# NVlabs/latentfusion

Hardware: AMD Instinct MI355X
Metric: pose-optim iters/sec (reconstruct+render+backward), 16 views, 128^3 voxels (higher is better)
Workload: dtype f32

## Files before the change

### latentfusion_amd/csrc/conv.hip

```cpp
#include "lf_common.h"

namespace {

constexpr int TX = 16;

template <int DIMS> struct TileGeom;
template <> struct TileGeom<3> { static constexpr int TY = 4, TZ = 4, HY = 6, HZ = 6, TAPS = 27; };
template <> struct TileGeom<2> { static constexpr int TY = 16, TZ = 1, HY = 18, HZ = 1, TAPS = 9; };

template <int NT, int NR, bool WHOLE = false>
__device__ __forceinline__ void epilogue_store(f32x4 (&acc)[NT][NR], const long (&rowoff)[NR], const long (&rowidx)[NR],
                                               const float* __restrict__ bias, float* __restrict__ y,
                                               float* __restrict__ norm_out, int Cout, int co_base,
                                               int ysc, long yss, bool vec_out,
                                               float he, unsigned flags, float slope, float eps,
                                               const float* __restrict__ prev_y = nullptr,
                                               const float* __restrict__ prev_norm = nullptr, unsigned prev_flags = 0,
                                               float* __restrict__ amax_out = nullptr) {
  float lane_amax = 0.f;
  const int lane = threadIdx.x & 63;
  const int cq = lane >> 4;
  float bv[NT][4];
#pragma unroll
  for (int t = 0; t < NT; ++t)
// ... 310 lines not shown
#pragma unroll
  for (int j = 0; j < 4; ++j) {
    const int r = wave * 4 + j;
    const int gy = y0 + ((DIMS == 3) ? (r & 3) : r);
    const int gz = (DIMS == 3) ? z0 + (r >> 2) : 0;
    const int gx = x0 + li;
    rowidx[j] = (gx < W && gy < H && gz < D) ? ((((long)n * D + gz) * H + gy) * W + gx) : -1;
    rowoff[j] = rowidx[j] < 0 ? -1 : rowidx[j] * Cout;
  }
  epilogue_store<1, 4>(acc, rowoff, rowidx, bias, y, norm_out, Cout, 0, 1 << 30, 0, (Cout & 3) == 0,
                       he, flags, slope, eps, prev_y, prev_norm, prev_flags);
}

namespace p3 {
constexpr int TZ = 4, TY = 8, HZ = 6, HY = 10, HX = TX + 2;
constexpr int HALO = HZ * HY * HX;
constexpr int NTHREADS = 512;
constexpr int NSLOT = (HALO * 4 + 63) / 64;
constexpr int NIT = (NSLOT + 7) / 8;
constexpr int BUF_FLOATS = NSLOT * 256;
}

__global__ void __launch_bounds__(512, 2) conv3d_c16_persistent_kernel(
    const float* __restrict__ x, const float* __restrict__ wpack, const float* __restrict__ bias,
    float* __restrict__ y, float* __restrict__ norm_out,
    int N, int D, int H, int W, int tiles_x, int tiles_y, int tiles_z, int ntiles,
    float he, unsigned flags, float slope, float eps,
    const float* __restrict__ prev_y, const float* __restrict__ prev_norm, unsigned prev_flags) {
  __shared__ __attribute__((aligned(16))) float lds[2 * p3::BUF_FLOATS];

  const int tid = threadIdx.x, lane = tid & 63;
  const int wave = __builtin_amdgcn_readfirstlane(tid >> 6);
  const int li = lane & 15, cq = lane >> 4;

  const int per = (ntiles + gridDim.x - 1) / gridDim.x;
  const int t_begin = blockIdx.x * per;
  const int t_end = min(t_begin + per, ntiles);
  if (t_begin >= t_end) return;

  const long nvox = (long)D * H * W;
  const unsigned sample_bytes = (unsigned)(nvox * 64);

  int rel[p3::NIT];
  int lxyz[p3::NIT];
#pragma unroll
  for (int it = 0; it < p3::NIT; ++it) {
    const int e = (wave + 8 * it) * 64 + lane;
    int v = e >> 2;
    const int q = e & 3;
    const int lx = v % p3::HX; v /= p3::HX;
    const int ly = v % p3::HY;
    const int lz = v / p3::HY;
    const bool inside = e < p3::HALO * 4;
    rel[it] = ((lz * H + ly) * W + lx) * 64 + q * 16;
    lxyz[it] = inside ? (lx | (ly << 8) | (lz << 16)) : 0x7f7f7f;
  }

  f32x4 wreg[27];
  {
    const float* wl = wpack + li * 16 + cq * 4;
#pragma unroll
    for (int tap = 0; tap < 27; ++tap) wreg[tap] = *(const f32x4*)(wl + tap * 256);
  }
  f32x4 bv4 = (f32x4){0.f, 0.f, 0.f, 0.f};
  if (bias != nullptr) bv4 = *(const f32x4*)(bias + cq * 4);

  int rowoffs[4];
#pragma unroll
  for (int j = 0; j < 4; ++j) {
    const int r = wave * 4 + j;
    rowoffs[j] = (((r >> 3) * p3::HY + (r & 7)) * p3::HX + li) * 16 + cq * 4;
  }

  auto issue_dma = [&](int t, int buf) {
    int tt = t;
    const int bx = tt % tiles_x; tt /= tiles_x;
    const int by = tt % tiles_y; tt /= tiles_y;
    const int bz = tt % tiles_z; tt /= tiles_z;
    const int n = tt;
    const int ox = bx * TX - 1, oy = by * p3::TY - 1, oz = bz * p3::TZ - 1;
    const int tile_off = ((oz * H + oy) * W + ox) * 64;
    __amdgpu_buffer_rsrc_t rs = __builtin_amdgcn_make_buffer_rsrc((void*)(x + (long)n * nvox * 16), 0,
                                                                  sample_bytes, 0x00020000);
#pragma unroll
    for (int it = 0; it < p3::NIT; ++it) {
      const int s = wave + 8 * it;
      if (s < p3::NSLOT) {
        const int gx = ox + (lxyz[it] & 0xff), gy = oy + ((lxyz[it] >> 8) & 0xff), gz = oz + (lxyz[it] >> 16);
        const bool ok = (unsigned)gx < (unsigned)W && (unsigned)gy < (unsigned)H && (unsigned)gz < (unsigned)D;
        const int voff = ok ? (rel[it] + tile_off) : 0x7fffffff;
        __builtin_amdgcn_raw_ptr_buffer_load_lds(
            rs, (__attribute__((address_space(3))) void*)(lds + buf * p3::BUF_FLOATS + s * 256), 16, voff, 0, 0, 0);
      }
    }
  };

  issue_dma(t_begin, 0);
  asm volatile("s_waitcnt vmcnt(0)" ::: "memory");
  __syncthreads();

  f32x4 acc[4];

  f32x4 pyv[4];
  float pnv[4];
  auto prefetch_prev = [&](int t) {
    if (prev_y == nullptr) return;
    int tt = t;
    const int bx = tt % tiles_x; tt /= tiles_x;
    const int by = tt % tiles_y; tt /= tiles_y;
    const int bz = tt % tiles_z; tt /= tiles_z;
    const float* pybase = prev_y + (long)tt * nvox * 16;
    const float* pnbase = prev_norm ? prev_norm + (long)tt * nvox : nullptr;
    const int gx = bx * TX + li;
#pragma unroll
    for (int j = 0; j < 4; ++j) {
      const int r = wave * 4 + j;
      const int gz = bz * p3::TZ + (r >> 3), gy = by * p3::TY + (r & 7);
      const bool ok = gx < W && gy < H && gz < D;
      const int vox = ok ? (gz * H + gy) * W + gx : 0;
      pyv[j] = ok ? *(const f32x4*)(pybase + vox * 16 + cq * 4) : (f32x4){0.f, 0.f, 0.f, 0.f};
      pnv[j] = (ok && pnbase) ? pnbase[vox] : 1.f;
    }
  };

  auto compute = [&](int buf) {
    const float* base = lds + buf * p3::BUF_FLOATS;
#pragma unroll
    for (int j = 0; j < 4; ++j) acc[j] = (f32x4){0.f, 0.f, 0.f, 0.f};
    f32x4 bcur[4], bnext[4];
#pragma unroll
    for (int j = 0; j < 4; ++j) bcur[j] = *(const f32x4*)(base + rowoffs[j]);
#pragma unroll
    for (int tap = 0; tap < 27; ++tap) {
      if (tap + 1 < 27) {
        const int t1 = tap + 1;
        const int kx = t1 % 3, ky = (t1 / 3) % 3, kz = t1 / 9;
        const int toff = ((kz * p3::HY + ky) * p3::HX + kx) * 16;
#pragma unroll
        for (int j = 0; j < 4; ++j) bnext[j] = *(const f32x4*)(base + rowoffs[j] + toff);
      }
#pragma unroll
      for (int s4 = 0; s4 < 4; ++s4)
#pragma unroll
        for (int j = 0; j < 4; ++j)
          acc[j] = __builtin_amdgcn_mfma_f32_16x16x4f32(wreg[tap][s4], bcur[j][s4], acc[j], 0, 0, 0);
#pragma unroll
      for (int j = 0; j < 4; ++j) bcur[j] = bnext[j];
    }
  };

  auto epilogue = [&](int t) {
    int tt = t;
    const int bx = tt % tiles_x; tt /= tiles_x;
    const int by = tt % tiles_y; tt /= tiles_y;
    const int bz = tt % tiles_z; tt /= tiles_z;
    const int n = tt;
    float* ybase = y + (long)n * nvox * 16;
    float* nbase = norm_out ? norm_out + (long)n * nvox : nullptr;
    const int gx = bx * TX + li;
#pragma unroll
    for (int j = 0; j < 4; ++j) {
      const int r = wave * 4 + j;
      const int gz = bz * p3::TZ + (r >> 3), gy = by * p3::TY + (r & 7);
      if (prev_y != nullptr) {
        const bool ok = gx < W && gy < H && gz < D;
        const int vox = ok ? (gz * H + gy) * W + gx : 0;
        const f32x4 yp = pyv[j];
        f32x4 g = acc[j] * he;
        if (prev_flags & LF_EPI_PIXELNORM) {
          float dot = g[0] * yp[0] + g[1] * yp[1] + g[2] * yp[2] + g[3] * yp[3];
          dot += __shfl_xor(dot, 16, 64);
          dot += __shfl_xor(dot, 32, 64);
          dot *= (1.f / 16.f);
          const float rinv = 1.0f / pnv[j];
#pragma unroll
          for (int e = 0; e < 4; ++e) g[e] = (g[e] - yp[e] * dot) * rinv;
        }
        if (prev_flags & LF_EPI_LRELU) {
#pragma unroll
          for (int e = 0; e < 4; ++e) g[e] = yp[e] > 0.f ? g[e] : g[e] * slope;
        }
        if (ok) *(f32x4*)(ybase + vox * 16 + cq * 4) = g;
        continue;
      }
      f32x4 v;
      float ss = 0.f;
#pragma unroll
      for (int e = 0; e < 4; ++e) {
        float u = acc[j][e] * he + bv4[e];
        if (flags & LF_EPI_LRELU) u = fmaxf(u, u * slope);
        v[e] = u;
        ss += u * u;
      }
      float r_ = 1.f;
      if (flags & LF_EPI_PIXELNORM) {
        ss += __shfl_xor(ss, 16, 64);
        ss += __shfl_xor(ss, 32, 64);
        r_ = sqrtf(ss / 16.f + eps);
        const float rinv = 1.0f / r_;
        v[0] *= rinv; v[1] *= rinv; v[2] *= rinv; v[3] *= rinv;
      }
      if (gx < W && gy < H && gz < D) {
        const int vox = (gz * H + gy) * W + gx;
        *(f32x4*)(ybase + vox * 16 + cq * 4) = v;
        if ((flags & LF_EPI_PIXELNORM) && nbase != nullptr && cq == 0) nbase[vox] = r_;
      }
    }
  };

  int cur = 0;
  if (wave < 4) {
    for (int t = t_begin; t < t_end; ++t) {
      if (t + 1 < t_end) issue_dma(t + 1, cur ^ 1);
      prefetch_prev(t);
      compute(cur);
      epilogue(t);
      asm volatile("s_waitcnt vmcnt(0)" ::: "memory");
      __syncthreads();
      cur ^= 1;
    }
  } else {
    for (int t = t_begin; t < t_end; ++t) {
      if (t + 1 < t_end) issue_dma(t + 1, cur ^ 1);
      if (t > t_begin) epilogue(t - 1);
      prefetch_prev(t);
      compute(cur);
      asm volatile("s_waitcnt vmcnt(0)" ::: "memory");
      __syncthreads();
      cur ^= 1;
    }
    epilogue(t_end - 1);
  }
}

template <int NT>
__global__ void __launch_bounds__(256) conv1x1_kernel(
    const float* __restrict__ x, const float* __restrict__ wpack, const float* __restrict__ bias,
    float* __restrict__ y, float* __restrict__ norm_out,
    int P, int Cin, int ksl, long x_batch_stride, long x_slice_stride, int Cout, int Kp,
    long y_batch_stride, int y_row_stride, int y_slice_channels, long y_slice_stride,
    float he, unsigned flags, float slope, float eps,
    const float* __restrict__ prev_y, const float* __restrict__ prev_norm, unsigned prev_flags,
    float* __restrict__ amax_out, const float* __restrict__ xscale) {
  const int tid = threadIdx.x, lane = tid & 63, wave = tid >> 6;
  const int li = lane & 15, cq = lane >> 4;
  const int n = blockIdx.z;
  const int co_base = blockIdx.y * NT * 16;
  const long p = (long)blockIdx.x * 64 + wave * 16 + li;
  const bool live = p < P;
  const bool vec_in = ((Cin & 3) == 0);
  const float* xrow = x + (long)n * x_batch_stride + (live ? p : 0) * Cin;
  const float* wrow = wpack + (long)(co_base + li) * Kp + cq * 4;

  f32x4 acc[NT][1];
#pragma unroll
  for (int t = 0; t < NT; ++t) acc[t][0] = (f32x4){0.f, 0.f, 0.f, 0.f};

  const int K = ksl * Cin;
  const int nchunks = Kp >> 4;
  auto load_b = [&](int kc) -> f32x4 {
    const int k0 = kc * 16 + cq * 4;
    f32x4 bfrag = (f32x4){0.f, 0.f, 0.f, 0.f};
    if (live && k0 < K) {
      const int s = k0 / Cin, c0 = k0 - s * Cin;
      const float* src = xrow + (long)s * x_slice_stride + c0;
      if (vec_in) {
        bfrag = *(const f32x4*)src;
        if (xscale != nullptr) bfrag = bfrag * xscale[((long)n * ksl + s) * P + p];
      } else {
#pragma unroll
        for (int e = 0; e < 4; ++e)
          if (k0 + e < K) bfrag[e] = src[e];
      }
    }
    return bfrag;
  };
  auto mac = [&](int kc, const f32x4& bfrag) {
#pragma unroll
    for (int t = 0; t < NT; ++t) {
      const f32x4 afrag = *(const f32x4*)(wrow + (long)t * 16 * Kp + kc * 16);
#pragma unroll
      for (int st = 0; st < 4; ++st)
        acc[t][0] = __builtin_amdgcn_mfma_f32_16x16x4f32(afrag[st], bfrag[st], acc[t][0], 0, 0, 0);
    }
  };
  int kc = 0;
  if (NT == 1) {
    for (; kc + 4 <= nchunks; kc += 4) {
      f32x4 b4[4];
#pragma unroll
      for (int u = 0; u < 4; ++u) b4[u] = load_b(kc + u);
#pragma unroll
      for (int u = 0; u < 4; ++u) mac(kc + u, b4[u]);
    }
  }
  for (; kc < nchunks; ++kc) mac(kc, load_b(kc));
  long rowidx[1] = {live ? ((long)n * P + p) : -1};
  long rowoff[1] = {live ? ((long)n * y_batch_stride + p * y_row_stride) : -1};
  const bool vec_out = ((y_row_stride | y_slice_channels) & 3) == 0 && ((y_batch_stride | y_slice_stride) & 3) == 0;
  epilogue_store<NT, 1>(acc, rowoff, rowidx, bias, y, norm_out, Cout, co_base, y_slice_channels, y_slice_stride,
                        vec_out, he, flags, slope, eps, prev_y, prev_norm, prev_flags, amax_out);
}

}

extern "C" int lf_conv3x3_cout_padded(int Cout) {
  lf_clear_error();
  const int c16 = (Cout + 15) & ~15;
  if (c16 <= 16) return 16;
  if (c16 <= 32) return 32;
  return (c16 + 63) & ~63;
}

extern "C" int lf_conv1x1_cout_padded(int Cout) {
  lf_clear_error();
  const int c16 = (Cout + 15) & ~15;
  if (c16 <= 16) return 16;
  if (c16 <= 32) return 32;
  if (c16 <= 64) return 64;
  return (c16 + 127) & ~127;
}

static int conv3x3_launch(const float* x, const float* wpack, const float* bias, float* y, float* norm_out,
                          int dims, int N, int D, int H, int W, int Cin, int Cout,
                          float he, unsigned flags, float slope, float eps, void* stream,
                          const float* prev_y, const float* prev_norm, unsigned prev_flags) {
  if (N <= 0 || D <= 0 || H <= 0 || W <= 0 || Cin <= 0 || Cout <= 0) return LF_EINVAL;
  if (prev_y != nullptr) {
    if (flags != 0 || bias != nullptr || (Cout != 16 && Cout != 32 && Cout != 64) || !lf_aligned16(prev_y)) return LF_EINVAL;
    if ((prev_flags & LF_EPI_PIXELNORM) && prev_norm == nullptr) return LF_EINVAL;
  }
  if (dims != 2 && dims != 3) return LF_EINVAL;
  if (dims == 2 && D != 1) return LF_EINVAL;
  if ((flags & LF_EPI_PIXELNORM) && Cout > 64) return LF_EINVAL;
  if (!lf_aligned16(x) || !lf_aligned16(y) || !lf_aligned16(wpack)) return LF_EALIGN;
  const int CinP = (Cin + 15) & ~15, CoutP = lf_conv3x3_cout_padded(Cout);
  const int ntiles = CoutP / 16;
  const int NT = ntiles >= 4 ? 4 : ntiles;
  const int groups = ntiles / NT;
  const int TY = dims == 3 ? 4 : 16, TZ = dims == 3 ? 4 : 1;
  const int tiles_x = (W + TX - 1) / TX, tiles_y = (H + TY - 1) / TY, tiles_z = (D + TZ - 1) / TZ;
  const long nblk = (long)tiles_x * tiles_y * tiles_z * N;
  if (nblk > 0x7fffffffL) return LF_EINVAL;
  dim3 grid((unsigned)nblk, groups), block(256);
  hipStream_t s = (hipStream_t)stream;
  if (Cin == 16 && Cout == 16 && dims == 3 && (long)D * H * W >= 4096 && (long)D * H * W * 64 < 0x7fffffffL &&
      slope > 0.f && slope < 1.f && (bias == nullptr || lf_aligned16(bias))) {
    const int ptx = (W + TX - 1) / TX, pty = (H + p3::TY - 1) / p3::TY, ptz = (D + p3::TZ - 1) / p3::TZ;
    const long pt = (long)ptx * pty * ptz * N;
    if (pt <= 0x7fffffffL) {
      const int cus = lf_cu_count();
      const unsigned pgrid = (unsigned)(pt < cus ? pt : cus);
      hipLaunchKernelGGL(conv3d_c16_persistent_kernel, dim3(pgrid), dim3(p3::NTHREADS), 0, s, x, wpack, bias, y, norm_out,
                         N, D, H, W, ptx, pty, ptz, (int)pt, he, flags, slope, eps, prev_y, prev_norm, prev_flags);
      return lf_launch_status();
    }
  }
  if (CinP == 16 && CoutP == 16) {
    if (dims == 3)
      hipLaunchKernelGGL((conv3x3_c16_kernel<3>), grid, block, 0, s, x, wpack, bias, y, norm_out, N, D, H, W, Cin, Cout,
                         tiles_x, tiles_y, tiles_z, he, flags, slope, eps, prev_y, prev_norm, prev_flags);
    else
      hipLaunchKernelGGL((conv3x3_c16_kernel<2>), grid, block, 0, s, x, wpack, bias, y, norm_out, N, D, H, W, Cin, Cout,
                         tiles_x, tiles_y, tiles_z, he, flags, slope, eps, prev_y, prev_norm, prev_flags);
    return lf_launch_status();
  }
#define LAUNCH(DM, T) hipLaunchKernelGGL((conv3x3_kernel<DM, T>), grid, block, 0, s, x, wpack, bias, y, norm_out, \
                                         N, D, H, W, Cin, Cout, CinP, CoutP, tiles_x, tiles_y, tiles_z, he, flags, slope, eps, \
                                         prev_y, prev_norm, prev_flags)
  if (dims == 3) { if (NT == 4) LAUNCH(3, 4); else if (NT == 2) LAUNCH(3, 2); else LAUNCH(3, 1); }
  else           { if (NT == 4) LAUNCH(2, 4); else if (NT == 2) LAUNCH(2, 2); else LAUNCH(2, 1); }
#undef LAUNCH
  return lf_launch_status();
}

extern "C" int lf_conv3x3_fwd(const float* x, const float* wpack, const float* bias, float* y, float* norm_out,
                              int dims, int N, int D, int H, int W, int Cin, int Cout,
                              float he, unsigned flags, float slope, float eps, void* stream) {
  lf_clear_error();
  return conv3x3_launch(x, wpack, bias, y, norm_out, dims, N, D, H, W, Cin, Cout, he, flags, slope, eps, stream,
                        nullptr, nullptr, 0);
}

extern "C" int lf_conv3x3_bwd_data(const float* gy, const float* wpack_t, float* gx, int dims, int N, int D, int H, int W,
                                   int Cin, int Cout, float he, const float* prev_y, const float* prev_norm,
                                   unsigned prev_flags, float slope, void* stream) {
  lf_clear_error();
  return conv3x3_launch(gy, wpack_t, nullptr, gx, nullptr, dims, N, D, H, W, Cin, Cout, he, 0, slope, 0.f, stream,
                        prev_y, prev_norm, prev_flags);
}

static int conv1x1_launch(const float* x, const float* wpack, const float* bias, float* y, float* norm_out,
                          int N, int P, int Cin, int ksl, long x_batch_stride, long x_slice_stride,
                          int Cout, long y_batch_stride, int y_row_stride, int y_slice_channels,
                          long y_slice_stride,
                          float he, unsigned flags, float slope, float eps, void* stream,
                          const float* prev_y, const float* prev_norm, unsigned prev_flags, float* amax_out = nullptr,
                          const float* xscale = nullptr) {
  if (N <= 0 || P <= 0 || Cin <= 0 || ksl <= 0 || Cout <= 0 || y_slice_channels <= 0) return LF_EINVAL;
  if (xscale != nullptr && (Cin & 3)) return LF_EALIGN;
  if (prev_y != nullptr) {
    if (flags != 0 || bias != nullptr || y_slice_channels != 16 || y_row_stride != 16 || (Cout & 15) ||
        !lf_aligned16(prev_y) || ((y_batch_stride | y_slice_stride) & 15))
      return LF_EINVAL;
    if ((prev_flags & LF_EPI_PIXELNORM) && prev_norm == nullptr) return LF_EINVAL;
    if ((prev_flags & LF_EPI_DOT) && (prev_flags != LF_EPI_DOT || prev_norm == nullptr)) return LF_EINVAL;
  }
  if (y_row_stride < (y_slice_channels < Cout ? y_slice_channels : Cout)) return LF_EINVAL;
  if (ksl > 1 && (Cin & 3)) return LF_EALIGN;
  if ((flags & LF_EPI_PIXELNORM) && Cout > 128) return LF_EINVAL;
  if (!lf_aligned16(x) || !lf_aligned16(y) || !lf_aligned16(wpack)) return LF_EALIGN;
  if (y == nullptr && !(prev_y != nullptr && (prev_flags & LF_EPI_DOT))) return LF_EINVAL;
  if ((Cin & 3) == 0 && ((x_batch_stride | x_slice_stride) & 3)) return LF_EALIGN;
  const int K = ksl * Cin, Kp = (K + 15) & ~15;
  const int CoutP = lf_conv1x1_cout_padded(Cout);
  const int ntiles = CoutP / 16;
  const int NT = ntiles >= 8 ? ((prev_y != nullptr && ntiles >= 16) ? 4 : 8) : ntiles;
  const int groups = ntiles / NT;
  dim3 grid((unsigned)((P + 63) / 64), groups, N), block(256);
  hipStream_t s = (hipStream_t)stream;
#define LAUNCH(T) hipLaunchKernelGGL((conv1x1_kernel<T>), grid, block, 0, s, x, wpack, bias, y, norm_out, \
                                     P, Cin, ksl, x_batch_stride, x_slice_stride, Cout, Kp, y_batch_stride, y_row_stride, \
                                     y_slice_channels, y_slice_stride, he, flags, slope, eps, prev_y, prev_norm, prev_flags, \
                                     amax_out, xscale)
  switch (NT) {
    case 1: LAUNCH(1); break;
    case 2: LAUNCH(2); break;
    case 4: LAUNCH(4); break;
    case 8: LAUNCH(8); break;
    default: return LF_EINVAL;
  }
#undef LAUNCH
  return lf_launch_status();
}

extern "C" int lf_conv1x1_fwd(const float* x, const float* wpack, const float* bias, float* y, float* norm_out,
                              int N, int P, int Cin, int ksl, long x_batch_stride, long x_slice_stride,
                              int Cout, long y_batch_stride, int y_row_stride, int y_slice_channels,
                              long y_slice_stride,
                              float he, unsigned flags, float slope, float eps, void* stream) {
  lf_clear_error();
  return conv1x1_launch(x, wpack, bias, y, norm_out, N, P, Cin, ksl, x_batch_stride, x_slice_stride, Cout,
                        y_batch_stride, y_row_stride, y_slice_channels, y_slice_stride, he, flags, slope, eps, stream,
                        nullptr, nullptr, 0);
}

extern "C" int lf_conv1x1_fwd_scaled(const float* x, const float* xscale, const float* wpack, const float* bias, float* y,
                                     float* norm_out, int N, int P, int Cin, int ksl, long x_batch_stride, long x_slice_stride,
                                     int Cout, long y_batch_stride, int y_row_stride, int y_slice_channels, long y_slice_stride,
                                     float he, unsigned flags, float slope, float eps, void* stream) {
  lf_clear_error();
  if (xscale == nullptr) return LF_EINVAL;
  return conv1x1_launch(x, wpack, bias, y, norm_out, N, P, Cin, ksl, x_batch_stride, x_slice_stride, Cout,
                        y_batch_stride, y_row_stride, y_slice_channels, y_slice_stride, he, flags, slope, eps, stream,
                        nullptr, nullptr, 0, nullptr, xscale);
}

extern "C" int lf_conv1x1_bwd_data(const float* gy, const float* wpack_t, float* gx, int N, int P, int Cin, int Cout,
                                   long y_batch_stride, int y_row_stride, int y_slice_channels, long y_slice_stride,
                                   float he, const float* prev_y, const float* prev_norm, unsigned prev_flags,
                                   float slope, float* amax_out, void* stream) {
  lf_clear_error();
  return conv1x1_launch(gy, wpack_t, nullptr, gx, nullptr, N, P, Cin, 1, (long)P * Cin, 0, Cout, y_batch_stride,
                        y_row_stride, y_slice_channels, y_slice_stride, he, 0, slope, 0.f, stream, prev_y, prev_norm,
                        prev_flags, amax_out);
}
```

### latentfusion_amd/csrc/lf_common.h

```cpp
#pragma once
#include <hip/hip_runtime.h>
#include <stdint.h>
#include "../../include/lf_hip.h"
#include "../../include/lf_hip_experimental.h"

#define LF_WAVE 64

typedef float f32x4 __attribute__((ext_vector_type(4)));

static inline void lf_clear_error() { (void)hipGetLastError(); }

static inline int lf_launch_status() {
  hipError_t e = hipGetLastError();
  return (int)e;
}

static inline bool lf_aligned16(const void* p) { return (((uintptr_t)p) & 15u) == 0; }

#include <atomic>
typedef std::atomic<unsigned long long> lf_devmask_t;
static inline hipError_t lf_ensure_dyn_lds(lf_devmask_t& done, const void* fn, int bytes) {
  int dev = 0;
  if (hipGetDevice(&dev) != hipSuccess) dev = 0;
  const unsigned long long bit = 1ull << (dev & 63);
  if (done.load(std::memory_order_acquire) & bit) return hipSuccess;
  const hipError_t e = hipFuncSetAttribute(fn, hipFuncAttributeMaxDynamicSharedMemorySize, bytes);
  if (e == hipSuccess) done.fetch_or(bit, std::memory_order_release);
  return e;
}

static inline int lf_cu_count() {
  static std::atomic<int> cus[64];
  int dev = 0, v = 0;
  const bool known = hipGetDevice(&dev) == hipSuccess;
  std::atomic<int>& slot = cus[dev & 63];
  const int c = slot.load(std::memory_order_relaxed);
  if (c != 0) return c;
  const int n = (known && hipDeviceGetAttribute(&v, hipDeviceAttributeMultiprocessorCount, dev) == hipSuccess && v > 0) ? v : 256;
  slot.store(n, std::memory_order_relaxed);
  return n;
}

__device__ __forceinline__ float lf_wave_sum(float v) {
#pragma unroll
  for (int o = 32; o > 0; o >>= 1) v += __shfl_xor(v, o, 64);
  return v;
}

#define LF_AMAX_SLOTS 64
#define LF_AMAX_STRIDE 32
static_assert(LF_AMAX_FLOATS == LF_AMAX_SLOTS * LF_AMAX_STRIDE, "lf_hip.h: LF_AMAX_FLOATS");

__device__ __forceinline__ void lf_amax_publish(float* base, float wave_max, int lane) {
  if (lane == 0 && wave_max > 0.f)
    atomicMax((unsigned int*)(base + (blockIdx.x % LF_AMAX_SLOTS) * LF_AMAX_STRIDE), __float_as_uint(wave_max));
}

__device__ __forceinline__ float lf_amax_read(const float* base, int lane) {
  float m = base[(lane % LF_AMAX_SLOTS) * LF_AMAX_STRIDE];
#pragma unroll
  for (int o = 32; o > 0; o >>= 1) m = fmaxf(m, __shfl_xor(m, o, 64));
  return m;
}

__device__ __forceinline__ float lf_lrelu(float v, float slope) { return v > 0.f ? v : v * slope; }

int lf_internal_ring_bf16_set_wgs(int v);
int lf_internal_wino_set_pack(int v);
int lf_internal_wino_set_forms(int v);
int lf_internal_fused_set_cfg(int v);
int lf_internal_splat_set_variant(int v);
int lf_internal_splat_set_chunk_cap(int v);
```

### latentfusion_amd/csrc/resample.hip

```cpp
#include "resample_map.h"

namespace {

typedef unsigned u32x4_t __attribute__((ext_vector_type(4)));

struct Tap {
  int x0, y0, z0, x1, y1, z1;
  float tx, ty, tz;
  float mx, my, mz;
};

__device__ __forceinline__ float lattice01(int i, int size, float step) {
  return (i < size / 2) ? step * (float)i : 1.f - step * (float)(size - 1 - i);
}


template <int KIND>
__device__ __forceinline__ void eval_grid(const float* __restrict__ cf, int x, int y, int z,
                                          int W, int H, int D, Steps st, float& gx, float& gy, float& gz,
                                          float& a, float& b, float& k) {
  a = lattice01(x, W, st.w);
  b = lattice01(y, H, st.h);
  k = lattice01(z, D, st.d);
  if (KIND == LF_MAP_O2C) {
// ... 213 lines not shown
    if (o[0] == 0xffffffffu) continue;
    const u32 b00 = o[0] + co, b01 = b00 + o[2], b10 = b00 + o[3], b11 = b01 + o[3];
    const f32x4 v000 = ldrec(rs, b00), v001 = ldrec(rs, b00 + o[1]), v010 = ldrec(rs, b01), v011 = ldrec(rs, b01 + o[1]);
    const f32x4 v100 = ldrec(rs, b10), v101 = ldrec(rs, b10 + o[1]), v110 = ldrec(rs, b11), v111 = ldrec(rs, b11 + o[1]);
    const float wx1 = f[0], wx0 = 1.f - f[0], wy1 = f[1], wy0 = 1.f - f[1], wz1 = f[2], wz0 = 1.f - f[2];
    const float w000 = wx0 * wy0 * wz0, w001 = wx1 * wy0 * wz0, w010 = wx0 * wy1 * wz0, w011 = wx1 * wy1 * wz0;
    const float w100 = wx0 * wy0 * wz1, w101 = wx1 * wy0 * wz1, w110 = wx0 * wy1 * wz1, w111 = wx1 * wy1 * wz1;
    f32x4 r;
#pragma unroll
    for (int e = 0; e < 4; ++e) {
      float acc = v000[e] * w000;
      asm("v_fmac_f32 %0, %1, %2" : "+v"(acc) : "v"(v001[e]), "v"(w001));
      asm("v_fmac_f32 %0, %1, %2" : "+v"(acc) : "v"(v010[e]), "v"(w010));
      asm("v_fmac_f32 %0, %1, %2" : "+v"(acc) : "v"(v011[e]), "v"(w011));
      asm("v_fmac_f32 %0, %1, %2" : "+v"(acc) : "v"(v100[e]), "v"(w100));
      asm("v_fmac_f32 %0, %1, %2" : "+v"(acc) : "v"(v101[e]), "v"(w101));
      asm("v_fmac_f32 %0, %1, %2" : "+v"(acc) : "v"(v110[e]), "v"(w110));
      asm("v_fmac_f32 %0, %1, %2" : "+v"(acc) : "v"(v111[e]), "v"(w111));
      r[e] = acc;
    }
    const int x = x0 + (vi & 3), y = y0 + ((vi >> 2) & 3), z = z0 + (vi >> 4);
    __builtin_amdgcn_raw_buffer_store_b128(__builtin_bit_cast(u32x4_t, r), ro, (int)((u32)((z * H + y) * W + x) * 64u + co), 0, 2);
  }
}

#include "resample_staged.inc"

#ifdef STAGED_TPW_OVERRIDE
constexpr int STAGED_TPW = STAGED_TPW_OVERRIDE;
#else
constexpr int STAGED_TPW = 16;
#endif

int g_bwd_coef_variant = 10;
int g_resample_variant = 3;

}

struct FwdPlan {
  bool vec;
  int lpt, tlx, tly, tlz, nbz;
  dim3 grid;
  Steps st;
};
static int fwd_plan(const float* vol, const float* out, int N, int D, int H, int W, int C, FwdPlan& p) {
  if ((long)D * H * W >= 0x7fffffffL) return LF_EINVAL;
  p.vec = (C % 4 == 0) && lf_aligned16(vol) && lf_aligned16(out);
  const int lpv = p.vec ? C / 4 : C;
  p.lpt = lpv < 256 ? lpv : 256;
  int lg = 0;
  while ((2 << lg) * p.lpt <= 256) ++lg;
  if (lg >= 6) { p.tlx = (lg + 2) / 3; p.tly = (lg + 1) / 3; p.tlz = lg / 3; }
  else         { p.tlx = lg < 2 ? lg : 2; p.tly = lg - p.tlx < 2 ? lg - p.tlx : 2; p.tlz = lg - p.tlx - p.tly; }
  p.nbz = (D + (1 << p.tlz) - 1) >> p.tlz;
  const int nby = (H + (1 << p.tly) - 1) >> p.tly;
  if ((long)p.nbz * N > 65535 || nby > 65535) return LF_EINVAL;
  p.grid = dim3((unsigned)((W + (1 << p.tlx) - 1) >> p.tlx), (unsigned)nby, (unsigned)(p.nbz * N));
  p.st = make_steps(D, H, W);
  return 0;
}

extern "C" int lf_resample3d_fwd(const float* vol, int vol_n, const float* coef, int kind, float* out,
                                 int N, int D, int H, int W, int C, void* stream) {
  lf_clear_error();
  if (N <= 0 || D <= 0 || H <= 0 || W <= 0 || C <= 0) return LF_EINVAL;
  if (vol_n != 1 && vol_n != N) return LF_EINVAL;
  if (kind != LF_MAP_O2C && kind != LF_MAP_C2O) return LF_EINVAL;
  const long bstride = vol_n == 1 ? 0 : (long)D * H * W * C;
  FwdPlan p;
  if (int e = fwd_plan(vol, out, N, D, H, W, C, p)) return e;
  hipStream_t s = (hipStream_t)stream;
  if (g_resample_variant == 4 && p.vec && C == 16 && (long)D * H * W * 64 < 0xffffffffL && W <= 65535) {
    const int ntx = (W + LT_X - 1) / LT_X, nty = (H + LT_Y - 1) / LT_Y, ntz = (D + LT_Z - 1) / LT_Z;
    const long nwg = (long)ntx * nty * ntz * N;
    if (nwg > 0x7fffffffL) return LF_EINVAL;
    LAUNCH_BY_KIND(resample_fwd_staged_kernel, dim3((unsigned)nwg), vol, bstride, coef, out, D, H, W, ntx, nty, ntz, p.st);
    return lf_launch_status();
  }
  if (g_resample_variant == 5 && p.vec && C == 16 && (long)D * H * W * 64 < 0xffffffffL) {
    const int nbz4 = (D + 3) >> 2, nbx16 = (W + 15) >> 4, nby4 = (H + 3) >> 2;
    if ((long)nbz4 * N > 65535 || nby4 > 65535) return LF_EINVAL;
    dim3 g5((unsigned)nbx16, (unsigned)nby4, (unsigned)(nbz4 * N));
    LAUNCH_BY_KIND(resample_fwd_c16_dedup_kernel, g5, vol, bstride, coef, out, D, H, W, nbx16, nby4, nbz4, p.st);
    return lf_launch_status();
  }
  if (g_resample_variant >= 3 && p.vec && C == 16 && (long)D * H * W * 64 < 0xffffffffL) {
    LAUNCH_BY_KIND(resample_fwd_c16_kernel, p.grid, vol, bstride, coef, out, D, H, W, p.nbz, p.st);
  } else if (g_resample_variant >= 2 && p.vec && (long)D * H * W * C * 4 < 0xffffffffL) {
    LAUNCH_BY_KIND(resample_fwd_lean_kernel, p.grid, vol, bstride, coef, out, D, H, W, C, p.lpt, p.tlx, p.tly, p.tlz, p.nbz, p.st);
  } else {
#define LAUNCH(K, V) hipLaunchKernelGGL((resample_fwd_kernel<K, V>), p.grid, dim3(256), 0, s, vol, bstride, coef, out, N, D, H, W, C, p.lpt, p.tlx, p.tly, p.tlz, p.nbz, p.st)
    if (kind == LF_MAP_O2C) { if (p.vec) LAUNCH(LF_MAP_O2C, 4); else LAUNCH(LF_MAP_O2C, 1); }
    else                    { if (p.vec) LAUNCH(LF_MAP_C2O, 4); else LAUNCH(LF_MAP_C2O, 1); }
#undef LAUNCH
  }
  return lf_launch_status();
}

static long staged_bwd_blocks(int D, int H, int W) {
  const long nt = (long)((W + LT_X - 1) / LT_X) * ((H + LT_Y - 1) / LT_Y) * ((D + LT_Z - 1) / LT_Z);
  return (nt + STAGED_TPW - 1) / STAGED_TPW;
}

static size_t bwd_coef_scratch_bytes(int N, int part_n, int D, int H, int W) {
  const long nvox = (long)D * H * W;
  const int vpb = bwd_vox_per_block(nvox, part_n);
  const BwdTile bt = bwd_tile(vpb, D, H, W);
  const long nblk = (long)bt.ntx * bt.nty * bt.ntz;
  const long nblk_staged = staged_bwd_blocks(D, H, W);
  return (size_t)N * (nblk > nblk_staged ? nblk : nblk_staged) * 18 * sizeof(float);
}

extern "C" size_t lf_resample3d_bwd_coef_scratch_bytes(int N, int D, int H, int W) {
  return bwd_coef_scratch_bytes(N, N, D, H, W);
}

extern "C" size_t lf_resample3d_bwd_coef_part_scratch_bytes(int N, int part_n, int D, int H, int W) {
  if (N <= 0 || part_n <= 0) return 0;
  return bwd_coef_scratch_bytes(N, part_n, D, H, W);
}

struct BwdCoefPlan {
  long nvox;
  int vpb, nblk, lpv;
  BwdTile bt;
  bool vec;
  dim3 grid;
  Steps st;
};
static int bwd_coef_plan(const float* gout, const float* vol, size_t scratch_bytes, int N, int part_n, int D, int H, int W, int C,
                         BwdCoefPlan& p) {
  if (scratch_bytes < bwd_coef_scratch_bytes(N, part_n, D, H, W)) return LF_ENOSPC;
  if ((long)D * H * W >= 0x7fffffffL) return LF_EINVAL;
  p.nvox = (long)D * H * W;
  p.vpb = bwd_vox_per_block(p.nvox, part_n);
  p.bt = bwd_tile(p.vpb, D, H, W);
  const long nblk_l = (long)p.bt.ntx * p.bt.nty * p.bt.ntz;
  if (nblk_l * N > 0x7fffffffL) return LF_EINVAL;
  p.nblk = (int)nblk_l;
  p.grid = dim3((unsigned)(nblk_l * N));
  p.vec = (C % 4 == 0) && lf_aligned16(gout) && lf_aligned16(vol);
  const int groups = p.vec ? C / 4 : C;
  p.lpv = 1;
  while (p.lpv < groups) p.lpv <<= 1;
  if (p.lpv > 64) return LF_EINVAL;
  p.st = make_steps(D, H, W);
  return 0;
}

static int bwd_coef_finish(const float* partial, int nblk, float* gcoef, int N, hipStream_t s) {
  if (int e = lf_launch_status()) return e;
  hipLaunchKernelGGL(resample_bwd_coef_reduce, dim3(N), dim3(256), 0, s, partial, nblk, gcoef);
  return lf_launch_status();
}

static int bwd_coef_launch(const float* gout, const float* vol, int vol_n, const float* coef,
                           float* gcoef, void* scratch, size_t scratch_bytes,
                           int N, int part_n, int D, int H, int W, int C, void* stream) {
  if (N <= 0 || D <= 0 || H <= 0 || W <= 0 || C <= 0) return LF_EINVAL;
  if (vol_n != 1 && vol_n != N) return LF_EINVAL;
  BwdCoefPlan p;
  if (int e = bwd_coef_plan(gout, vol, scratch_bytes, N, part_n, D, H, W, C, p)) return e;
  const long bstride = vol_n == 1 ? 0 : p.nvox * C;
  hipStream_t s = (hipStream_t)stream;
  float* partial = (float*)scratch;
  if (g_resample_variant == 4 && p.vec && C == 16 && p.nvox * 64 < 0xffffffffL && W <= 65535) {
    const int ntx = (W + LT_X - 1) / LT_X, nty = (H + LT_Y - 1) / LT_Y, ntz = (D + LT_Z - 1) / LT_Z;
    const long nb = staged_bwd_blocks(D, H, W);
    if (nb * N > 0x7fffffffL) return LF_EINVAL;
    hipLaunchKernelGGL((resample_bwd_coef_staged_kernel<STAGED_TPW>), dim3((unsigned)(nb * N)), dim3(256), 0, s, gout, vol, bstride, coef,
                       partial, (int)nb, D, H, W, ntx, nty, ntz, p.st);
    return bwd_coef_finish(partial, (int)nb, gcoef, N, s);
  }
  if (g_resample_variant >= 2 && p.vec && C == 16 && p.vpb >= 64 && p.nvox * 64 < 0xffffffffL) {
    const int v = g_bwd_coef_variant;
    const bool big = p.vpb >= 256;
#define LAUNCH(...) hipLaunchKernelGGL((__VA_ARGS__), p.grid, dim3(256), 0, s, gout, vol, bstride, coef, partial, p.nblk, p.vpb, p.bt, D, H, W, p.st)
    if (v == 1)              LAUNCH(resample_bwd_coef_c16_kernel<1, 1>);
    else if (v == 2)         LAUNCH(resample_bwd_coef_c16_kernel<1, 2>);
    else if (v == 3)         LAUNCH(resample_bwd_coef_c16_kernel<4, 2>);
    else if (v == 6 && big)  LAUNCH(resample_bwd_coef_c16_dedup_kernel<2, 1>);
    else if (v == 7 && big)  LAUNCH(resample_bwd_coef_c16_dedup_kernel<1, 1>);
    else if (v == 8 && big)  LAUNCH(resample_bwd_coef_c16_dedup_kernel<2, 4>);
    else if (v == 9 && big)  LAUNCH(resample_bwd_coef_c16_dedup_kernel<1, 5>);
    else if (v == 10 && big) LAUNCH(resample_bwd_coef_c16_dedup_kernel<2, 1, true>);
    else if (v == 11 && big) LAUNCH(resample_bwd_coef_c16_dedup_kernel<1, 1, true>);
    else if (v == 4)         LAUNCH(resample_bwd_coef_c16_kernel<6, 1>);
    else                     LAUNCH(resample_bwd_coef_c16_kernel<8, 1>);
#undef LAUNCH
  } else if (p.vec) {
    hipLaunchKernelGGL((resample_bwd_coef_kernel<4>), p.grid, dim3(256), 0, s, gout, vol, bstride, coef, partial, p.nblk, p.vpb, p.bt, N, D, H, W, C, p.lpv, p.st);
  } else {
    hipLaunchKernelGGL((resample_bwd_coef_kernel<1>), p.grid, dim3(256), 0, s, gout, vol, bstride, coef, partial, p.nblk, p.vpb, p.bt, N, D, H, W, C, p.lpv, p.st);
  }
  return bwd_coef_finish(partial, p.nblk, gcoef, N, s);
}

extern "C" int lf_resample3d_bwd_coef(const float* gout, const float* vol, int vol_n, const float* coef,
                                      float* gcoef, void* scratch, size_t scratch_bytes,
                                      int N, int D, int H, int W, int C, void* stream) {
  lf_clear_error();
  return bwd_coef_launch(gout, vol, vol_n, coef, gcoef, scratch, scratch_bytes, N, N, D, H, W, C, stream);
}

extern "C" int lf_resample3d_bwd_coef_part(const float* gout, const float* vol, int vol_n, const float* coef,
                                           float* gcoef, void* scratch, size_t scratch_bytes,
                                           int N, int D, int H, int W, int C, int part_n, void* stream) {
  lf_clear_error();
  if (!gout || !vol || !coef || !gcoef || !scratch) return LF_EINVAL;
  if (part_n <= 0 || N <= 0) return LF_EINVAL;
  return bwd_coef_launch(gout, vol, vol_n, coef, gcoef, scratch, scratch_bytes, N, part_n, D, H, W, C, stream);
}

extern "C" int lf_resample3d_fwd_indexed(const float* vol, int vol_n, const int* vol_idx, const float* coef, int kind, float* out,
                                         int N, int D, int H, int W, int C, void* stream) {
  lf_clear_error();
  if (!vol || !vol_idx || !coef || !out) return LF_EINVAL;
  if (N <= 0 || D <= 0 || H <= 0 || W <= 0 || C <= 0 || vol_n < 1) return LF_EINVAL;
  if (kind != LF_MAP_O2C && kind != LF_MAP_C2O) return LF_EINVAL;
  if (((uintptr_t)vol_idx & 3) != 0) return LF_EALIGN;
  const long bstride = (long)D * H * W * C;
  FwdPlan p;
  if (int e = fwd_plan(vol, out, N, D, H, W, C, p)) return e;
  hipStream_t s = (hipStream_t)stream;
  if (g_resample_variant >= 3 && p.vec && C == 16 && (long)D * H * W * 64 < 0xffffffffL) {
    LAUNCH_BY_KIND(resample_fwd_c16_indexed_kernel, p.grid, vol, bstride, vol_idx, vol_n, coef, out, D, H, W, p.nbz, p.st);
  } else if (g_resample_variant >= 2 && p.vec && (long)D * H * W * C * 4 < 0xffffffffL) {
    LAUNCH_BY_KIND(resample_fwd_lean_indexed_kernel, p.grid, vol, bstride, vol_idx, vol_n, coef, out, D, H, W, C, p.lpt, p.tlx, p.tly, p.tlz, p.nbz, p.st);
  } else {
#define LAUNCH(K, V) hipLaunchKernelGGL((resample_fwd_indexed_kernel<K, V>), p.grid, dim3(256), 0, s, vol, bstride, vol_idx, vol_n, coef, out, N, D, H, W, C, p.lpt, p.tlx, p.tly, p.tlz, p.nbz, p.st)
    if (kind == LF_MAP_O2C) { if (p.vec) LAUNCH(LF_MAP_O2C, 4); else LAUNCH(LF_MAP_O2C, 1); }
    else                    { if (p.vec) LAUNCH(LF_MAP_C2O, 4); else LAUNCH(LF_MAP_C2O, 1); }
#undef LAUNCH
  }
  return lf_launch_status();
}

extern "C" size_t lf_resample3d_bwd_coef_indexed_scratch_bytes(int N, int part_n, int D, int H, int W) {
  if (N <= 0 || part_n <= 0) return 0;
  return bwd_coef_scratch_bytes(N, part_n, D, H, W);
}

extern "C" int lf_resample3d_bwd_coef_indexed(const float* gout, const float* vol, int vol_n, const int* vol_idx, const float* coef,
                                              float* gcoef, void* scratch, size_t scratch_bytes,
                                              int N, int D, int H, int W, int C, int part_n, void* stream) {
  lf_clear_error();
  if (!gout || !vol || !vol_idx || !coef || !gcoef || !scratch) return LF_EINVAL;
  if (part_n <= 0 || N <= 0 || vol_n < 1) return LF_EINVAL;
  if (D <= 0 || H <= 0 || W <= 0 || C <= 0) return LF_EINVAL;
  if (((uintptr_t)vol_idx & 3) != 0) return LF_EALIGN;
  BwdCoefPlan p;
  if (int e = bwd_coef_plan(gout, vol, scratch_bytes, N, part_n, D, H, W, C, p)) return e;
  const long bstride = p.nvox * C;
  hipStream_t s = (hipStream_t)stream;
  float* partial = (float*)scratch;
  if (g_resample_variant >= 2 && p.vec && C == 16 && p.vpb >= 64 && p.nvox * 64 < 0xffffffffL) {
    if (p.vpb >= 256)
      hipLaunchKernelGGL((resample_bwd_coef_c16_dedup_indexed_kernel<2, 1, true>), p.grid, dim3(256), 0, s, gout, vol, bstride, vol_idx, vol_n, coef, partial, p.nblk, p.vpb, p.bt, D, H, W, p.st);
    else
      hipLaunchKernelGGL((resample_bwd_coef_c16_indexed_kernel<8, 1>), p.grid, dim3(256), 0, s, gout, vol, bstride, vol_idx, vol_n, coef, partial, p.nblk, p.vpb, p.bt, D, H, W, p.st);
  } else if (p.vec) {
    hipLaunchKernelGGL((resample_bwd_coef_indexed_kernel<4>), p.grid, dim3(256), 0, s, gout, vol, bstride, vol_idx, vol_n, coef, partial, p.nblk, p.vpb, p.bt, N, D, H, W, C, p.lpv, p.st);
  } else {
    hipLaunchKernelGGL((resample_bwd_coef_indexed_kernel<1>), p.grid, dim3(256), 0, s, gout, vol, bstride, vol_idx, vol_n, coef, partial, p.nblk, p.vpb, p.bt, N, D, H, W, C, p.lpv, p.st);
  }
  return bwd_coef_finish(partial, p.nblk, gcoef, N, s);
}

extern "C" int lf_resample3d_bwd_vol(const float* gout, const float* coef, int kind, float* gvol, int vol_n,
                                     int N, int D, int H, int W, int C, void* stream) {
  lf_clear_error();
  if (N <= 0 || D <= 0 || H <= 0 || W <= 0 || C <= 0) return LF_EINVAL;
  if (vol_n != 1 && vol_n != N) return LF_EINVAL;
  const long bstride = vol_n == 1 ? 0 : (long)D * H * W * C;
  const long items = (long)D * H * W * C;
  dim3 grid((unsigned)min((items + 255) / 256, (long)65535 * 16), N), block(256);
  hipStream_t s = (hipStream_t)stream;
  if (kind == LF_MAP_O2C)
    hipLaunchKernelGGL((resample_bwd_vol_kernel<LF_MAP_O2C>), grid, block, 0, s, gout, coef, gvol, bstride, N, D, H, W, C, make_steps(D, H, W));
  else if (kind == LF_MAP_C2O)
    hipLaunchKernelGGL((resample_bwd_vol_kernel<LF_MAP_C2O>), grid, block, 0, s, gout, coef, gvol, bstride, N, D, H, W, C, make_steps(D, H, W));
  else
    return LF_EINVAL;
  return lf_launch_status();
}

#ifdef STAGE_TS
extern "C" int lf_debug_stage_ts(void* dst) {
  return (int)hipMemcpyFromSymbol(dst, HIP_SYMBOL(g_stage_ts), sizeof(unsigned long long) * 256 * 16, 0, hipMemcpyDeviceToHost);
}
#endif

extern "C" int lf_set_tuning(int key, int value) {
  if (key == 1) {
    const int prev = g_resample_variant;
    if (value >= 1 && value <= 5) g_resample_variant = value;
    return prev;
  }
  if (key == 4) return lf_internal_splat_set_variant(value);
  if (key == 6) return lf_internal_splat_set_chunk_cap(value);
  if (key == 3) return lf_internal_fused_set_cfg(value);
  if (key == 7) return lf_internal_wino_set_pack(value);
  if (key == 8) return lf_internal_wino_set_forms(value);
  if (key == 5) return lf_internal_ring_bf16_set_wgs(value);
  if (key == 2) {
    const int prev = g_bwd_coef_variant;
    if (value >= 1 && value <= 11) g_bwd_coef_variant = value;
    return prev;
  }
  return LF_EINVAL;
}

extern "C" int lf_resample3d_fwd_io(const void* vol, int vol_n, const float* coef, int kind, void* out,
                                    int N, int D, int H, int W, int io, void* stream) {
  lf_clear_error();
  if (N <= 0 || D <= 0 || H <= 0 || W <= 0 || io < 0 || io > 3) return LF_EINVAL;
  if ((vol_n != 1 && vol_n != N) || (kind != LF_MAP_O2C && kind != LF_MAP_C2O)) return LF_EINVAL;
  if (!lf_aligned16(vol) || !lf_aligned16(out)) return LF_EALIGN;
  if ((long)D * H * W * 64 >= 0xffffffffL) return LF_EINVAL;
  const long bstride = vol_n == 1 ? 0 : (long)D * H * W * 16;
  const int nbz4 = (D + 3) >> 2;
  if ((long)nbz4 * N > 65535 || ((H + 3) >> 2) > 65535) return LF_EINVAL;
  dim3 g4((unsigned)((W + 3) >> 2), (unsigned)((H + 3) >> 2), (unsigned)(nbz4 * N)), block(256);
  const Steps st = make_steps(D, H, W);
  typedef void (*kern_t)(const float*, long, const float*, float*, int, int, int, int, Steps);
  static const kern_t kerns[2][4] = {
      {resample_fwd_c16_kernel<LF_MAP_O2C, 0>, resample_fwd_c16_kernel<LF_MAP_O2C, 1>, resample_fwd_c16_kernel<LF_MAP_O2C, 2>, resample_fwd_c16_kernel<LF_MAP_O2C, 3>},
      {resample_fwd_c16_kernel<LF_MAP_C2O, 0>, resample_fwd_c16_kernel<LF_MAP_C2O, 1>, resample_fwd_c16_kernel<LF_MAP_C2O, 2>, resample_fwd_c16_kernel<LF_MAP_C2O, 3>}};
  hipLaunchKernelGGL(kerns[kind == LF_MAP_O2C ? 0 : 1][io], g4, block, 0, (hipStream_t)stream, (const float*)vol, bstride, coef, (float*)out, D, H, W, nbz4, st);
  return lf_launch_status();
}
```

Before: 198.7.

## Add specialized double-buffered kernel for 16-channel projection 1x1 backward-data

Adds a dedicated kernel for the 1x1 conv backward-data path when Cin is 16 and the previous layer used LReLU plus pixel-norm. Each wave handles one batch/pixel group and walks the depth slices with a double-buffered prefetch of activations, norms and weights. It fuses MFMA, the pixel-norm backward and the LReLU backward into one epilogue. It is persistent-grid launched and on by default with a tuning key, replacing the generic conv1x1 launch for this shape, at the cost of extra code and register use.

Result: no change. 198.5 (-0.1%).

```diff
diff --git a/latentfusion_amd/csrc/conv.hip b/latentfusion_amd/csrc/conv.hip
--- a/latentfusion_amd/csrc/conv.hip
+++ b/latentfusion_amd/csrc/conv.hip
@@ -636,6 +636,95 @@
                         vec_out, he, flags, slope, eps, prev_y, prev_norm, prev_flags, amax_out);
 }
 
+constexpr int PBS_H = 4;
+
+__device__ __forceinline__ f32x4 proj_bwd_epilogue(const f32x4 acc, const f32x4 yp, float nr, float he, float slope) {
+#pragma clang fp contract(off)
+  f32x4 g;
+#pragma unroll
+  for (int e = 0; e < 4; ++e) g[e] = __builtin_fmaf(he, acc[e], 0.f);
+  float dot = __builtin_fmaf(g[3], yp[3], __builtin_fmaf(g[2], yp[2], __builtin_fmaf(g[0], yp[0], g[1] * yp[1])));
+  dot += __shfl_xor(dot, 16, 64);
+  dot += __shfl_xor(dot, 32, 64);
+  dot *= (1.f / 16.f);
+  const float rinv = 1.0f / nr;
+#pragma unroll
+  for (int e = 0; e < 4; ++e) g[e] = __builtin_fmaf(-yp[e], dot, g[e]) * rinv;
+#pragma unroll
+  for (int e = 0; e < 4; ++e) g[e] = yp[e] > 0.f ? g[e] : g[e] * slope;
+  return g;
+}
+
+struct PbsSet { f32x4 yp[PBS_H], af[PBS_H]; float nr[PBS_H]; };
+
+__global__ void __launch_bounds__(256, 4) proj_bwd_block_kernel(
+    const float* __restrict__ gy, const float* __restrict__ wpack_t, float* __restrict__ gx,
+    const float* __restrict__ prev_y, const float* __restrict__ prev_norm,
+    int N, int P, int D, long y_batch_stride, unsigned y_slice_stride, int groups, int jobs, int reverse,
+    float he, float slope) {
+  const int lane = threadIdx.x & 63, li = lane & 15, cq = lane >> 4;
+  const int nwaves = gridDim.x * 4;
+  const int Dm = D - D % (2 * PBS_H);
+  for (int job = blockIdx.x * 4 + (threadIdx.x >> 6); job < jobs; job += nwaves) {
+    const int ns = job / groups, grp = job - ns * groups;
+    const int n = reverse ? N - 1 - ns : ns;
+    const int p = grp * 16 + li;
+    const bool live = p < P;
+    const int pe = live ? p : P - 1;
+    const f32x4 b = *(const f32x4*)(gy + ((long)n * P + pe) * 16 + cq * 4);
+    const float* ybase = prev_y + (long)n * y_batch_stride;
+    const float* nbase = prev_norm + (long)n * (y_batch_stride >> 4);
+    float* obase = gx + (long)n * y_batch_stride;
+    unsigned wofs = (unsigned)(li * 16 + cq * 4);
+    asm volatile("" : "+v"(wofs));
+    const float* wrow = wpack_t + wofs;
+    const unsigned off0 = (unsigned)pe * 16u + (unsigned)cq * 4u;
+    auto request = [&](PbsSet& s, int d0) {
+#pragma unroll
+      for (int i = 0; i < PBS_H; ++i) {
+        const unsigned dd = (unsigned)min(d0 + i, D - 1);
+        const unsigned off = off0 + dd * y_slice_stride;
+        s.yp[i] = *(const f32x4*)(ybase + off);
+        s.nr[i] = nbase[off >> 4];
+        s.af[i] = *(const f32x4*)(wrow + dd * 256u);
+      }
+    };
+    auto consume = [&](const PbsSet& s, int i, int d) {
+      f32x4 acc = (f32x4){0.f, 0.f, 0.f, 0.f};
+#pragma unroll
+      for (int st = 0; st < 4; ++st) acc = __builtin_amdgcn_mfma_f32_16x16x4f32(s.af[i][st], b[st], acc, 0, 0, 0);
+      const f32x4 g = proj_bwd_epilogue(acc, s.yp[i], s.nr[i], he, slope);
+      if (live) *(f32x4*)(obase + (off0 + (unsigned)d * y_slice_stride)) = g;
+    };
+    PbsSet sa, sb;
+    request(sa, 0);
+    for (int d0 = 0; d0 < Dm; d0 += 2 * PBS_H) {
+      request(sb, d0 + PBS_H);
+#pragma unroll
+      for (int i = 0; i < PBS_H; ++i) consume(sa, i, d0 + i);
+      request(sa, d0 + 2 * PBS_H);
+#pragma unroll
+      for (int i = 0; i < PBS_H; ++i) consume(sb, i, d0 + PBS_H + i);
+    }
+    const int rem = D - Dm;
+    if (rem > PBS_H) request(sb, Dm + PBS_H);
+#pragma unroll
+    for (int i = 0; i < PBS_H; ++i)
+      if (i < rem) consume(sa, i, Dm + i);
+#pragma unroll
+    for (int i = 0; i < PBS_H; ++i)
+      if (PBS_H + i < rem) consume(sb, i, Dm + PBS_H + i);
+  }
+}
+
+int g_proj_bwd_mode = 1;
+
+}
+
+int lf_internal_proj_bwd_set_mode(int v) {
+  const int prev = g_proj_bwd_mode;
+  if (v >= 0 && v <= 2) g_proj_bwd_mode = v;
+  return prev;
 }
 
 extern "C" int lf_conv3x3_cout_padded(int Cout) {
@@ -795,6 +884,21 @@
                                    float he, const float* prev_y, const float* prev_norm, unsigned prev_flags,
                                    float slope, float* amax_out, void* stream) {
   lf_clear_error();
+  if (g_proj_bwd_mode != 0 && N > 0 && P > 0 && Cin == 16 && Cout > 0 && (Cout & 15) == 0 && y_slice_channels == 16 &&
+      y_row_stride == 16 && prev_y != nullptr && prev_norm != nullptr && prev_flags == (LF_EPI_LRELU | LF_EPI_PIXELNORM) &&
+      amax_out == nullptr && gx != nullptr && lf_aligned16(gy) && lf_aligned16(wpack_t) && lf_aligned16(gx) && lf_aligned16(prev_y) &&
+      lf_aligned16(prev_norm) && y_batch_stride > 0 && y_slice_stride > 0 && ((y_batch_stride | y_slice_stride) & 15) == 0) {
+    const int D = Cout / 16;
+    const long last = ((long)P - 1) * 16 + ((long)D - 1) * y_slice_stride + 16;
+    const long groups = ((long)P + 15) / 16, jobs = groups * N;
+    if (last * 4 < 0x7fffffffL && jobs < 0x7fffffffL) {
+      const long wgs = (jobs + 3) / 4, cap = (long)lf_cu_count() * 4;
+      hipLaunchKernelGGL(proj_bwd_block_kernel, dim3((unsigned)(wgs < cap ? wgs : cap)), dim3(256), 0, (hipStream_t)stream, gy, wpack_t,
+                         gx, prev_y, prev_norm, N, P, D, y_batch_stride, (unsigned)y_slice_stride, (int)groups, (int)jobs,
+                         g_proj_bwd_mode == 2 ? 1 : 0, he, slope);
+      return lf_launch_status();
+    }
+  }
   return conv1x1_launch(gy, wpack_t, nullptr, gx, nullptr, N, P, Cin, 1, (long)P * Cin, 0, Cout, y_batch_stride,
                         y_row_stride, y_slice_channels, y_slice_stride, he, 0, slope, 0.f, stream, prev_y, prev_norm,
                         prev_flags, amax_out);
diff --git a/latentfusion_amd/csrc/lf_common.h b/latentfusion_amd/csrc/lf_common.h
--- a/latentfusion_amd/csrc/lf_common.h
+++ b/latentfusion_amd/csrc/lf_common.h
@@ -68,6 +68,7 @@
 int lf_internal_ring_bf16_set_wgs(int v);
 int lf_internal_wino_set_pack(int v);
 int lf_internal_wino_set_forms(int v);
+int lf_internal_proj_bwd_set_mode(int v);
 int lf_internal_fused_set_cfg(int v);
 int lf_internal_splat_set_variant(int v);
 int lf_internal_splat_set_chunk_cap(int v);
diff --git a/latentfusion_amd/csrc/resample.hip b/latentfusion_amd/csrc/resample.hip
--- a/latentfusion_amd/csrc/resample.hip
+++ b/latentfusion_amd/csrc/resample.hip
@@ -539,6 +539,7 @@
   if (key == 3) return lf_internal_fused_set_cfg(value);
   if (key == 7) return lf_internal_wino_set_pack(value);
   if (key == 8) return lf_internal_wino_set_forms(value);
+  if (key == 9) return lf_internal_proj_bwd_set_mode(value);
   if (key == 5) return lf_internal_ring_bf16_set_wgs(value);
   if (key == 2) {
     const int prev = g_bwd_coef_variant;
```
